# Rorisis/Co-Occ

Hardware: AMD Instinct MI355X
Metric: samples/sec (6-cam frame + sweep -> occ+render), 200x200x16 grid (higher is better)
Workload: dtype f32 (split-f16 products, fp32 accumulate)

## Files before the change

co_occ_amd/csrc/gemm_h2.hip:

```cpp
#include <stdlib.h>
#include <string.h>
#include <type_traits>

#include "conv_k.h"

#include "h2_rows.h"

typedef float f32x16 __attribute__((ext_vector_type(16)));
typedef _Float16 f16x8 __attribute__((ext_vector_type(8)));

__device__ __forceinline__ void glds16_(const void* g, void* l) {
  __builtin_amdgcn_global_load_lds((const __attribute__((address_space(1))) void*)g, (__attribute__((address_space(3))) void*)l,
                                   16, 0, 0);
}

__device__ __forceinline__ void h2_epilogue_vec(const ConvK& p, size_t orow, int n, f32x4 v) {
  if (p.res_mode == 3) v = v + *(const f32x4*)(p.res + orow * p.res_stride + n);
  if (p.scale) v = v * *(const f32x4*)(p.scale + n);
  if (p.bias) v = v + *(const f32x4*)(p.bias + n);
  if (p.res_mode == 1) v = v + *(const f32x4*)(p.res + orow * p.res_stride + n);
  if (p.relu && (p.relu == 1 || n < p.relu)) { v[0] = fmaxf(v[0], 0.f); v[1] = fmaxf(v[1], 0.f); v[2] = fmaxf(v[2], 0.f); v[3] = fmaxf(v[3], 0.f); }
  if (p.res_mode == 2) v = v * *(const f32x4*)(p.res + orow * p.res_stride + n);
  if (p.out_h2) { store_h2(p.out, orow, p.out_stride, n, v); h2_guard(p.h2_flag, v); }
  else *(f32x4*)(p.out + orow * p.out_stride + n) = v;
// ... 492 lines not shown
    p2(STC{}, I1{});
    H2_FENCE();
  };
  if (nsteps > 0) {
    issueA(0);
    loadB(I0{});
  }
  __syncthreads();
  if (nsteps > 0) {
    load_frag(I0{}, I0{}, I0{});
    if (TERMS == 1) load_frag(I1{}, I0{}, I1{});
  }
  for (int st = 0; st < nsteps; st += 2) {
    step(I0{}, st + 1 < nsteps);
    if (st + 1 < nsteps) step(I1{}, st + 2 < nsteps);
  }

  const int nb = n0 + wave * 32 + 4 * h;
  const float alpha = p.alpha_dev ? p.alpha * *p.alpha_dev : p.alpha, lo = TERMS == 3 ? alpha * (1.f / H2_LO_SCALE) : 0.f;
  if (p.splitk > 1) {
#pragma unroll
    for (int i = 0; i < TM; ++i) {
      const int m = m0 + i * 32 + li;
      if (m >= p.M) continue;
      float* o = p.ws + ((size_t)blockIdx.y * p.M + m) * p.Npad + nb;
#pragma unroll
      for (int j = 0; j < 4; ++j) {
        f32x4 v;
#pragma unroll
        for (int e = 0; e < 4; ++e) v[e] = (TERMS == 3 ? hh[i][4 * j + e] * alpha + xx[i][4 * j + e] * lo : hh[i][4 * j + e] * alpha);
        if (p.tile_sem) st_agent(o + 8 * j, v);
        else *(f32x4*)(o + 8 * j) = v;
      }
    }
    if (p.tile_sem && h2_splitk_arrive(p, mtile * p.ntiles + nt)) h2_splitk_reduce<TM>(p, m0, nb, li);
  } else {
    const bool vec = (p.Cout & 3) == 0 && (p.out_stride & 3) == 0 && (!p.res || (p.res_stride & 3) == 0);
#pragma unroll
    for (int i = 0; i < TM; ++i) {
      const int m = m0 + i * 32 + li;
      if (m >= p.M) continue;
      const size_t orow = p.out_rows ? (size_t)p.out_rows[m] : (size_t)m;
#pragma unroll
      for (int j = 0; j < 4; ++j) {
        const int n = nb + 8 * j;
        if (n >= p.Cout) continue;
        f32x4 v;
#pragma unroll
        for (int e = 0; e < 4; ++e) v[e] = (TERMS == 3 ? hh[i][4 * j + e] * alpha + xx[i][4 * j + e] * lo : hh[i][4 * j + e] * alpha);
        if (vec) {
          h2_epilogue_vec(p, orow, n, v);
        } else {
#pragma unroll
          for (int e = 0; e < 4; ++e)
            if (n + e < p.Cout) p.out[orow * p.out_stride + n + e] = epilogue(p, v[e], n + e, orow);
        }
      }
    }
  }
}

template <int NCW>
__global__ __launch_bounds__(256, NCW == 4 ? 3 : 2) void k_gemm_h2n(ConvK p) {
  constexpr int BM = NCW == 4 ? 64 : 256, TM = NCW == 2 ? 4 : 2, NJ = BM / 32;
  constexpr unsigned STAGE = BM * 128;
  __shared__ __attribute__((aligned(16))) char As[2 * BM * 128];

  const int mtiles = (p.M + BM - 1) / BM;
  const int mtile = blockIdx.x;
  if (mtile >= mtiles) return;
  const int m0 = mtile * BM;
  if (p.M_dev) {
    p.M = min(p.M, *p.M_dev);
    if (m0 >= p.M) return;
  }
  const int tid = threadIdx.x;
  const int wave = __builtin_amdgcn_readfirstlane(tid >> 6), lane = tid & 63;
  const int li = lane & 31, h = lane >> 5;
  const int srow = lane >> 3, slot = lane & 7;
  const int colblk = NCW == 4 ? wave : (NCW == 2 ? (wave & 1) : 0);
  const int rowbase = NCW == 4 ? 0 : (NCW == 2 ? (wave >> 1) * 128 : wave * 64);
  const int taps = p.taps;
  const long long rowbytes = (long long)p.in_stride * 4;
  const char* inb = (const char*)p.in;
  const char* zrow = (const char*)p.zrow;
  const unsigned aq = (unsigned)((slot ^ ((4 * (wave & 1) + (srow >> 1)) & 7)) * 16);
  int rix[NJ];
#pragma unroll
  for (int j = 0; j < NJ; ++j) {
    const int m = m0 + (j * 4 + wave) * 8 + srow;
    rix[j] = m < p.M ? m : -1;
  }
  const int nsteps = p.total_iters;
  int ckc = 0, ct = 0;
  const long long wstep = (long long)(p.Npad >> 5) * 4096;
  const char* wcur = (const char*)p.w + (long long)colblk * 4096 + lane * 16;
  const int gstride = p.gstride;
  int tnext[NJ];
  auto tload = [&]() {
#pragma unroll
    for (int j = 0; j < NJ; ++j) tnext[j] = rix[j] >= 0 ? p.gather[(size_t)ct * gstride + rix[j]] : -1;
  };
  if (nsteps > 0) tload();
  auto issueA = [&](int buf) {
    const long long coff = (long long)ckc * 128 + aq;
#pragma unroll
    for (int j = 0; j < NJ; ++j) {
      const char* src = tnext[j] >= 0 ? inb + ((long long)tnext[j] * rowbytes + coff) : zrow;
      glds16_(src, &As[buf * STAGE + (j * 4 + wave) * 8 * 128]);
    }
    if (++ct == taps) { ct = 0; ++ckc; }
    tload();
  };
  f16x8 breg[2][2][2];
  auto loadB = [&](auto bufc) {
    constexpr int B_ = decltype(bufc)::value;
#pragma unroll
    for (int s = 0; s < 2; ++s)
#pragma unroll
      for (int pl = 0; pl < 2; ++pl) breg[B_][s][pl] = *(const f16x8*)(wcur + (s * 2 + pl) * 1024);
    wcur += wstep;
  };
  unsigned fragoff[4];
#pragma unroll
  for (int q = 0; q < 4; ++q) {
    const int sl = (q & 1) * 4 + 2 * (q >> 1) + h;
    fragoff[q] = (rowbase + li) * 128 + ((sl ^ ((li >> 1) & 7)) << 4);
  }
  f16x8 fr[2][TM];
  auto load_frag = [&](auto bufc, auto stagec, auto qc) {
    constexpr int BUF = decltype(bufc)::value, ST = decltype(stagec)::value, Q = decltype(qc)::value;
#pragma unroll
    for (int i = 0; i < TM; ++i) fr[BUF][i] = *(const f16x8*)&As[fragoff[Q] + (ST * STAGE + i * 4096)];
  };
  auto load_plane = [&](auto planec, auto stagec, auto sc) {
    constexpr int PL = decltype(planec)::value, S_ = decltype(sc)::value;
    load_frag(planec, stagec, std::integral_constant<int, 2 * S_ + PL>{});
  };
  f32x16 hh[TM], xx[TM];
#pragma unroll
  for (int i = 0; i < TM; ++i)
#pragma unroll
    for (int r = 0; r < 16; ++r) { hh[i][r] = 0.f; xx[i][r] = 0.f; }
  auto p01 = [&](auto setc, auto sc) {
    constexpr int B_ = decltype(setc)::value, S_ = decltype(sc)::value;
#pragma unroll
    for (int i = 0; i < TM; ++i) hh[i] = __builtin_amdgcn_mfma_f32_32x32x16_f16(breg[B_][S_][0], fr[0][i], hh[i], 0, 0, 0);
#pragma unroll
    for (int i = 0; i < TM; ++i) xx[i] = __builtin_amdgcn_mfma_f32_32x32x16_f16(breg[B_][S_][1], fr[0][i], xx[i], 0, 0, 0);
  };
  auto p2 = [&](auto setc, auto sc) {
    constexpr int B_ = decltype(setc)::value, S_ = decltype(sc)::value;
#pragma unroll
    for (int i = 0; i < TM; ++i) xx[i] = __builtin_amdgcn_mfma_f32_32x32x16_f16(breg[B_][S_][0], fr[1][i], xx[i], 0, 0, 0);
  };
  using I0 = std::integral_constant<int, 0>; using I1 = std::integral_constant<int, 1>;
  auto step = [&](auto stc, bool more) {
    constexpr int ST = decltype(stc)::value;
    using STC = std::integral_constant<int, ST>; using SNC = std::integral_constant<int, ST ^ 1>;
    if (more) { issueA(ST ^ 1); loadB(SNC{}); }
    load_plane(I1{}, STC{}, I0{});
    p01(STC{}, I0{});
    H2_FENCE();
    load_plane(I0{}, STC{}, I1{});
    p2(STC{}, I0{});
    H2_FENCE();
    load_plane(I1{}, STC{}, I1{});
    p01(STC{}, I1{});
    H2_FENCE();
    __syncthreads();
    if (more) load_plane(I0{}, SNC{}, I0{});
    p2(STC{}, I1{});
    H2_FENCE();
  };
  if (nsteps > 0) {
    issueA(0);
    loadB(I0{});
  }
  __syncthreads();
  if (nsteps > 0) load_frag(I0{}, I0{}, I0{});
  for (int st = 0; st < nsteps; st += 2) {
    step(I0{}, st + 1 < nsteps);
    if (st + 1 < nsteps) step(I1{}, st + 2 < nsteps);
  }

  const int nb = colblk * 32 + 4 * h;
  const float alpha = p.alpha_dev ? p.alpha * *p.alpha_dev : p.alpha, lo = alpha * (1.f / H2_LO_SCALE);
  const bool vec = (p.Cout & 3) == 0 && (p.out_stride & 3) == 0 && (!p.res || (p.res_stride & 3) == 0);
#pragma unroll
  for (int i = 0; i < TM; ++i) {
    const int m = m0 + rowbase + i * 32 + li;
    if (m >= p.M) continue;
    const size_t orow = p.out_rows ? (size_t)p.out_rows[m] : (size_t)m;
#pragma unroll
    for (int j = 0; j < 4; ++j) {
      const int n = nb + 8 * j;
      if (n >= p.Cout) continue;
      f32x4 v;
#pragma unroll
      for (int e = 0; e < 4; ++e) v[e] = hh[i][4 * j + e] * alpha + xx[i][4 * j + e] * lo;
      if (vec) {
        h2_epilogue_vec(p, orow, n, v);
      } else {
#pragma unroll
        for (int e = 0; e < 4; ++e)
          if (n + e < p.Cout) p.out[orow * p.out_stride + n + e] = epilogue(p, v[e], n + e, orow);
      }
    }
  }
}

template <int NCH>
__global__ __launch_bounds__(256, 2) void k_gemm_h2p(ConvK p) {
  constexpr int BM = 128, TM = 4;
  constexpr unsigned STAGE = BM * 128;
  __shared__ __attribute__((aligned(16))) char As[NCH * BM * 128];
  const int id = blockIdx.x;
  int mtile, nt, slot_ = id >> 3;
  if (p.mtiles_per_xcd > 0) {
    const int xcd = id & 7;
    const int mt_local = slot_ / p.ntiles;
    nt = slot_ - mt_local * p.ntiles;
    mtile = xcd * p.mtiles_per_xcd + mt_local;
    if (mt_local >= p.mtiles_per_xcd || mtile >= p.mtiles) return;
  } else {
    mtile = id / p.ntiles;
    nt = id - mtile * p.ntiles;
  }
  const int m0 = mtile * BM, n0 = nt * 128;
  const int tid = threadIdx.x;
  const int wave = __builtin_amdgcn_readfirstlane(tid >> 6), lane = tid & 63;
  const int li = lane & 31, h = lane >> 5;
  const int srow = lane >> 3, slot = lane & 7;
  const long long rowbytes = (long long)p.in_stride * 4;
  const char* inb = (const char*)p.in;
  const char* zrow = (const char*)p.zrow;
  const unsigned aq = (unsigned)((slot ^ ((4 * (wave & 1) + (srow >> 1)) & 7)) * 16);
#pragma unroll
  for (int c = 0; c < NCH; ++c)
#pragma unroll
    for (int j = 0; j < 4; ++j) {
      const int m = m0 + (j * 4 + wave) * 8 + srow;
      const char* src = m < p.M ? inb + ((long long)m * rowbytes + c * 128 + aq) : zrow;
      glds16_(src, &As[c * STAGE + (j * 4 + wave) * 8 * 128]);
    }
  f16x8 breg[NCH][2][2];
  const long long wstep = (long long)(p.Npad >> 5) * 4096;
  const char* wcur = (const char*)p.w + (long long)((n0 >> 5) + wave) * 4096 + lane * 16;
#pragma unroll
  for (int c = 0; c < NCH; ++c)
#pragma unroll
    for (int s2 = 0; s2 < 2; ++s2)
#pragma unroll
      for (int pl = 0; pl < 2; ++pl) breg[c][s2][pl] = *(const f16x8*)(wcur + c * wstep + (s2 * 2 + pl) * 1024);
  unsigned fragoff[4];
#pragma unroll
  for (int q = 0; q < 4; ++q) {
    const int sl = (q & 1) * 4 + 2 * (q >> 1) + h;
    fragoff[q] = li * 128 + ((sl ^ ((li >> 1) & 7)) << 4);
  }
  f32x16 hh[TM], xx[TM];
#pragma unroll
  for (int i = 0; i < TM; ++i)
#pragma unroll
    for (int r = 0; r < 16; ++r) { hh[i][r] = 0.f; xx[i][r] = 0.f; }
  __syncthreads();
#pragma unroll
  for (int c = 0; c < NCH; ++c) {
#pragma unroll
    for (int s2 = 0; s2 < 2; ++s2) {
      f16x8 fhi[TM], flo[TM];
#pragma unroll
      for (int i = 0; i < TM; ++i) {
        fhi[i] = *(const f16x8*)&As[fragoff[2 * s2 + 0] + (c * STAGE + i * 4096)];
        flo[i] = *(const f16x8*)&As[fragoff[2 * s2 + 1] + (c * STAGE + i * 4096)];
      }
#pragma unroll
      for (int i = 0; i < TM; ++i) hh[i] = __builtin_amdgcn_mfma_f32_32x32x16_f16(breg[c][s2][0], fhi[i], hh[i], 0, 0, 0);
#pragma unroll
      for (int i = 0; i < TM; ++i) xx[i] = __builtin_amdgcn_mfma_f32_32x32x16_f16(breg[c][s2][1], fhi[i], xx[i], 0, 0, 0);
#pragma unroll
      for (int i = 0; i < TM; ++i) xx[i] = __builtin_amdgcn_mfma_f32_32x32x16_f16(breg[c][s2][0], flo[i], xx[i], 0, 0, 0);
      H2_FENCE();
    }
  }
  const int nb = n0 + wave * 32 + 4 * h;
  const float alpha = p.alpha_dev ? p.alpha * *p.alpha_dev : p.alpha, lo = alpha * (1.f / H2_LO_SCALE);
#pragma unroll
  for (int i = 0; i < TM; ++i) {
    const int m = m0 + i * 32 + li;
    if (m >= p.M) continue;
#pragma unroll
    for (int j = 0; j < 4; ++j) {
      const int n = nb + 8 * j;
      if (n >= p.Cout) continue;
      f32x4 v;
#pragma unroll
      for (int e = 0; e < 4; ++e) v[e] = hh[i][4 * j + e] * alpha + xx[i][4 * j + e] * lo;
      h2_epilogue_vec(p, (size_t)m, n, v);
    }
  }
}

static int* g_h2_flag = nullptr;
int coocc_h2_flag_ptr(int** out) {
  if (!g_h2_flag) {
    void* p = nullptr;
    COOCC_HIP(hipHostMalloc(&p, 64, hipHostMallocMapped | hipHostMallocCoherent));
    memset(p, 0, 64);
    g_h2_flag = (int*)p;
  }
  *out = g_h2_flag;
  return COOCC_OK;
}
extern "C" int coocc_h2_overflow(int reset) {
  if (!g_h2_flag) return 0;
  const int v = *(volatile int*)g_h2_flag != 0;
  if (reset) *(volatile int*)g_h2_flag = 0;
  return v;
}
extern "C" int coocc_device_fault(int reset) {
  if (!g_h2_flag) return 0;
  const int v = ((volatile int*)g_h2_flag)[1];
  if (reset) ((volatile int*)g_h2_flag)[1] = 0;
  return v;
}

int coocc_launch_h2(ConvK& k, const coocc_conv_desc* d, hipStream_t s) {
  const bool one = d->mfma_dtype == 4;
  const int kc = one ? 64 : 32;
  COOCC_CHECK_ARG(d->Cin % kc == 0 && d->in_stride % kc == 0, "conv_fwd: H2 operands need Cin and in_stride % 32 == 0 (f16 operands: % 64)");
  COOCC_CHECK_ARG(!one || (d->wgroup_rows == 0 && !d->out_h2), "conv_fwd: the one-term f16 path has no weight groups / H2 output");
  COOCC_CHECK_ARG(d->wgroup_rows == 0 || d->wgroup_rows % 128 == 0, "conv_fwd: wgroup_rows must be a multiple of 128");
  const bool table = d->gather != nullptr;
  const bool zshare = !table && !d->out_rows && !d->M_dev && k.stride == 1 && k.Xo == k.Xi && k.Yo == k.Yi && k.Zo == k.Zi && k.kz >= 1 && k.kz <= 3 &&
                      (k.taps > 1 || d->wgroup_rows > 0);
  COOCC_CHECK_ARG(zshare || d->wgroup_rows == 0, "conv_fwd: weight groups need the stride-1 same geometry");
  k.kchunks = d->Cin / kc;
  k.total_iters = k.taps * k.kchunks;
  k.wgroup_floats = (size_t)k.taps * k.kchunks * k.Npad * 32;
  k.out16 = d->out16;
  k.out16_stride = d->out16_stride;
  COOCC_CHECK_ARG(!d->out16 || (d->Cout % 4 == 0 && d->out16_stride % 4 == 0 && !d->out_rows && ((uintptr_t)d->out16 & 7) == 0),
                  "conv_fwd: out16 needs Cout % 4 == 0, out16_stride % 4 == 0, no row scatter");
  k.alpha = d->alpha != 0.f ? d->alpha : 1.f;
  k.alpha_dev = d->alpha_dev;
  k.M_dev = d->M_dev;
  k.out_h2 = d->out_h2;
  COOCC_CHECK_ARG(!d->out_h2 || (d->Cout % 4 == 0 && d->out_stride % 32 == 0 && !d->out_rows),
                  "conv_fwd: out_h2 needs Cout % 4 == 0, out_stride % 32 == 0, no row scatter");
  k.out_h2t = d->out_h2_twin;
  COOCC_CHECK_ARG(!d->out_h2_twin || (!one && d->Cout % 32 == 0 && !d->out_rows && ((uintptr_t)d->out_h2_twin & 15) == 0 && (d->out_stride & 3) == 0 &&
                                      (!d->res || (d->res_stride & 3) == 0)),
                  "conv_fwd: out_h2_twin needs mfma_dtype 3, Cout % 32 == 0, 16-byte aligned rows, no row scatter");
  k.tile_sem = d->tile_sem;
  int rc = coocc_zero_row(&k.zrow);
  if (rc != COOCC_OK) return rc;
  rc = coocc_h2_flag_ptr(&k.h2_flag);
  if (rc != COOCC_OK) return rc;
  k.ntiles = (k.Cout + 127) / 128;
  k.mtiles = (k.M + 127) / 128;
  k.mtiles_per_xcd = k.mtiles >= 64 ? (k.mtiles + 7) / 8 : 0;
  const int gsz = zshare ? k.kz : 1;
  int splitk = d->splitk;
  const long long blocks = (long long)k.mtiles * k.ntiles;
  const int ngroups = k.total_iters / gsz;
  if (splitk <= 0) {
    splitk = 1;
    const bool vec4 = (d->Cout & 3) == 0 && (d->out_stride & 3) == 0 && (!d->res || (d->res_stride & 3) == 0) && (((uintptr_t)d->out) & 15) == 0;
    const bool second_pass_ok = vec4 || (!d->out_h2 && !d->out16 && !d->out_h2_twin);
    static const int target = getenv("COOCC_SPLITK_TARGET") ? atoi(getenv("COOCC_SPLITK_TARGET")) : 512;
    if (blocks < target / 2 && ngroups >= 8 && d->ws && !d->M_dev && (d->tile_sem ? true : (!d->out_rows && second_pass_ok))) {
      splitk = (int)(target / blocks);
      if (splitk > ngroups / 4) splitk = ngroups / 4;
      if (splitk > 64) splitk = 64;
      while (splitk > 1 && (long long)splitk * d->M * k.Npad > d->ws_floats) --splitk;
      if (splitk < 1) splitk = 1;
    }
  }
  int gps = (ngroups + splitk - 1) / splitk;
  k.iters_per_split = gps * gsz;
  k.splitk = (k.total_iters + k.iters_per_split - 1) / k.iters_per_split;
  COOCC_CHECK_ARG(k.splitk == 1 || (d->ws && !d->M_dev && (long long)k.splitk * d->M * k.Npad <= d->ws_floats),
                  "conv_fwd: split-K workspace too small (or split-K with a device row count)");
  COOCC_CHECK_ARG(k.splitk == 1 || d->tile_sem || (!d->out_h2 && !d->out16 && !d->out_h2_twin) ||
                      ((d->Cout & 3) == 0 && (d->out_stride & 3) == 0 && (!d->res || (d->res_stride & 3) == 0) && (((uintptr_t)d->out) & 15) == 0),
                  "conv_fwd: split-K with an H2 / f16 output needs 16-byte aligned rows (Cout, strides % 4 == 0)");
  COOCC_CHECK_ARG(k.splitk == 1 || !d->tile_sem || (long long)k.mtiles * k.ntiles <= d->tile_sem_ints,
                  "conv_fwd: tile_sem holds fewer counters than the launch has output tiles");
  dim3 grid(k.mtiles_per_xcd ? 8 * k.mtiles_per_xcd * k.ntiles : k.mtiles * k.ntiles, k.splitk);
  static const bool pointwise_on = !(getenv("COOCC_H2_POINTWISE") && atoi(getenv("COOCC_H2_POINTWISE")) == 0);
  if (pointwise_on && !zshare && !table && !one && k.taps == 1 && k.stride == 1 && k.px == 0 && k.py == 0 && k.pz == 0 && k.Xo == k.Xi &&
      k.Yo == k.Yi && k.Zo == k.Zi && k.kchunks <= 4 && k.splitk == 1 && !d->M_dev && !d->out_rows && blocks >= 256 &&
      (d->Cout & 3) == 0 && (d->out_stride & 3) == 0 && (!d->res || (d->res_stride & 3) == 0)) {
    switch (k.kchunks) {
      case 1: hipLaunchKernelGGL(k_gemm_h2p<1>, grid, dim3(256), 0, s, k); break;
      case 2: hipLaunchKernelGGL(k_gemm_h2p<2>, grid, dim3(256), 0, s, k); break;
      case 3: hipLaunchKernelGGL(k_gemm_h2p<3>, grid, dim3(256), 0, s, k); break;
      default: hipLaunchKernelGGL(k_gemm_h2p<4>, grid, dim3(256), 0, s, k); break;
    }
    COOCC_LAUNCH_CHECK("k_gemm_h2p");
    return COOCC_OK;
  }
  if (!zshare) {
    if (one) {
      if (table) hipLaunchKernelGGL((k_gemm_h2w<true, 1>), grid, dim3(256), 0, s, k);
      else hipLaunchKernelGGL((k_gemm_h2w<false, 1>), grid, dim3(256), 0, s, k);
    } else {
      const char* narrow_env = getenv("COOCC_H2_NARROW");
      const bool narrow_on = !(narrow_env && atoi(narrow_env) == 0);
      if (narrow_on && table && k.Cout <= 64 && k.ntiles == 1 && k.splitk == 1 && !d->tile_sem && (long long)k.mtiles >= 512) {
        const dim3 gridn((unsigned)((k.M + 255) / 256), 1);
        if (k.Cout <= 32) hipLaunchKernelGGL(k_gemm_h2n<1>, gridn, dim3(256), 0, s, k);
        else hipLaunchKernelGGL(k_gemm_h2n<2>, gridn, dim3(256), 0, s, k);
        COOCC_LAUNCH_CHECK("k_gemm_h2n");
        return COOCC_OK;
      }
      if (narrow_on && table && k.Cout > 96 && k.ntiles == 1 && k.splitk == 1 && !d->tile_sem && (long long)k.mtiles >= 128 && (long long)k.mtiles < 1024) {
        const dim3 gridn((unsigned)((k.M + 63) / 64), 1);
        hipLaunchKernelGGL(k_gemm_h2n<4>, gridn, dim3(256), 0, s, k);
        COOCC_LAUNCH_CHECK("k_gemm_h2n<4>");
        return COOCC_OK;
      }
      if (table) hipLaunchKernelGGL(k_gemm_h2w<true>, grid, dim3(256), 0, s, k);
      else hipLaunchKernelGGL(k_gemm_h2w<false>, grid, dim3(256), 0, s, k);
    }
    COOCC_LAUNCH_CHECK("k_gemm_h2w");
    return COOCC_OK;
  }
  COOCC_CHECK_ARG((long long)d->M < (1ll << 30) && (136ull + 2ull * ((unsigned long long)k.Yi + 2) * k.Zi) * d->in_stride * 4ull < 0xFFFFFF00ull,
                  "conv_fwd: the split-f16 kernel addresses a tile's window with 32-bit byte offsets");
  const bool xy = !(k.kx == 1 && k.ky == 1 && k.px == 0 && k.py == 0);
  if (one) {
    if (k.kz == 3) { if (xy) hipLaunchKernelGGL((k_gemm_h2z<3, true, 0, 1>), grid, dim3(256), 0, s, k); else hipLaunchKernelGGL((k_gemm_h2z<3, false, 0, 1>), grid, dim3(256), 0, s, k); }
    else if (k.kz == 2) { if (xy) hipLaunchKernelGGL((k_gemm_h2z<2, true, 0, 1>), grid, dim3(256), 0, s, k); else hipLaunchKernelGGL((k_gemm_h2z<2, false, 0, 1>), grid, dim3(256), 0, s, k); }
    else { if (xy) hipLaunchKernelGGL((k_gemm_h2z<1, true, 0, 1>), grid, dim3(256), 0, s, k); else hipLaunchKernelGGL((k_gemm_h2z<1, false, 0, 1>), grid, dim3(256), 0, s, k); }
    COOCC_LAUNCH_CHECK("k_gemm_h2z<f16>");
    return COOCC_OK;
  }
  static const int abl = getenv("COOCC_H2_ABLATE") ? atoi(getenv("COOCC_H2_ABLATE")) : 0;
  if (abl && !xy && k.kz == 3) {
    switch (abl) {
      case 1: hipLaunchKernelGGL((k_gemm_h2z<3, false, 1>), grid, dim3(256), 0, s, k); break;
      case 2: hipLaunchKernelGGL((k_gemm_h2z<3, false, 2>), grid, dim3(256), 0, s, k); break;
      case 4: hipLaunchKernelGGL((k_gemm_h2z<3, false, 4>), grid, dim3(256), 0, s, k); break;
      case 8: hipLaunchKernelGGL((k_gemm_h2z<3, false, 8>), grid, dim3(256), 0, s, k); break;
      case 7: hipLaunchKernelGGL((k_gemm_h2z<3, false, 7>), grid, dim3(256), 0, s, k); break;
      case 16: hipLaunchKernelGGL((k_gemm_h2z<3, false, 16>), grid, dim3(256), 0, s, k); break;
      case 24: hipLaunchKernelGGL((k_gemm_h2z<3, false, 24>), grid, dim3(256), 0, s, k); break;
      default: hipLaunchKernelGGL((k_gemm_h2z<3, false, 15>), grid, dim3(256), 0, s, k); break;
    }
    COOCC_LAUNCH_CHECK("k_gemm_h2z<ablation>");
    return COOCC_OK;
  }
  if (!xy) {
    if (k.kz == 3) hipLaunchKernelGGL((k_gemm_h2z<3, false>), grid, dim3(256), 0, s, k);
    else if (k.kz == 2) hipLaunchKernelGGL((k_gemm_h2z<2, false>), grid, dim3(256), 0, s, k);
    else hipLaunchKernelGGL((k_gemm_h2z<1, false>), grid, dim3(256), 0, s, k);
  } else {
    if (k.kz == 3) hipLaunchKernelGGL((k_gemm_h2z<3, true>), grid, dim3(256), 0, s, k);
    else if (k.kz == 2) hipLaunchKernelGGL((k_gemm_h2z<2, true>), grid, dim3(256), 0, s, k);
    else hipLaunchKernelGGL((k_gemm_h2z<1, true>), grid, dim3(256), 0, s, k);
  }
  COOCC_LAUNCH_CHECK("k_gemm_h2z");
  return COOCC_OK;
}

__global__ __launch_bounds__(256) void k_rows_to_h2(const float* __restrict__ in, int in_stride, long long rows, int C, float scale,
                                                     char* __restrict__ out, const int32_t* __restrict__ row_ids,
                                                     const int32_t* __restrict__ n_dev, int* __restrict__ flag,
                                                     const float* __restrict__ scale_dev) {
  if (n_dev) rows = min(rows, (long long)*n_dev);
  if (scale_dev) scale *= *scale_dev;
  const int c8 = C >> 3;
  const long long i = (long long)blockIdx.x * blockDim.x + threadIdx.x;
  if (i >= rows * c8) return;
  const long long r = i / c8;
  const int c = (int)(i - r * c8) * 8;
  const long long sr = row_ids ? (long long)row_ids[r] : r;
  const f32x4 a = *(const f32x4*)(in + sr * in_stride + c), b = *(const f32x4*)(in + sr * in_stride + c + 4);
  f16x8 hi, lo;
#pragma unroll
  for (int e = 0; e < 4; ++e) {
    _Float16 u, v;
    split_h2(a[e] * scale, u, v); hi[e] = u; lo[e] = v;
    split_h2(b[e] * scale, u, v); hi[4 + e] = u; lo[4 + e] = v;
  }
  char* o = out + r * (long long)C * 4 + (c >> 5) * 128 + (c & 31) * 2;
  *(f16x8*)o = hi;
  *(f16x8*)(o + 64) = lo;
  h2_guard(flag, a * scale);
  h2_guard(flag, b * scale);
}

extern "C" int coocc_rows_to_h2_ex(const float* in, int in_stride, int64_t rows, int C, float scale, const float* scale_dev,
                                   void* out_h2, void* stream) {
  COOCC_CHECK_ARG(in && out_h2 && rows >= 0 && C > 0 && C % 32 == 0 && in_stride % 4 == 0 && in_stride >= C, "rows_to_h2: bad args");
  COOCC_CHECK_ARG(((uintptr_t)in & 15) == 0 && ((uintptr_t)out_h2 & 15) == 0, "rows_to_h2: pointers must be 16-byte aligned");
  if (rows == 0) return COOCC_OK;
  int* flag = nullptr;
  if (coocc_h2_flag_ptr(&flag) != COOCC_OK) return COOCC_EHIP;
  hipLaunchKernelGGL(k_rows_to_h2, dim3(cdiv(rows * (C / 8), 256)), dim3(256), 0, as_stream(stream), in, in_stride, (long long)rows, C,
                     scale, (char*)out_h2, (const int32_t*)nullptr, (const int32_t*)nullptr, flag, scale_dev);
  COOCC_LAUNCH_CHECK("k_rows_to_h2");
  return COOCC_OK;
}

extern "C" int coocc_rows_to_h2(const float* in, int in_stride, int64_t rows, int C, float scale, void* out_h2, void* stream) {
  return coocc_rows_to_h2_ex(in, in_stride, rows, C, scale, nullptr, out_h2, stream);
}

extern "C" int coocc_rows_to_h2_gather(const float* in, int in_stride, const int32_t* row_ids, int64_t n_cap, const int32_t* n_dev,
                                       int C, float scale, void* out_h2, void* stream) {
  COOCC_CHECK_ARG(in && out_h2 && row_ids && n_cap >= 0 && C > 0 && C % 32 == 0 && in_stride % 4 == 0, "rows_to_h2_gather: bad args");
  COOCC_CHECK_ARG(((uintptr_t)in & 15) == 0 && ((uintptr_t)out_h2 & 15) == 0, "rows_to_h2_gather: pointers must be 16-byte aligned");
  if (n_cap == 0) return COOCC_OK;
  int* flag = nullptr;
  if (coocc_h2_flag_ptr(&flag) != COOCC_OK) return COOCC_EHIP;
  hipLaunchKernelGGL(k_rows_to_h2, dim3(cdiv(n_cap * (C / 8), 256)), dim3(256), 0, as_stream(stream), in, in_stride, (long long)n_cap, C,
                     scale, (char*)out_h2, row_ids, n_dev, flag, (const float*)nullptr);
  COOCC_LAUNCH_CHECK("k_rows_to_h2");
  return COOCC_OK;
}

__global__ __launch_bounds__(256) void k_rows_to_f16(const float* __restrict__ in, int in_stride, long long rows, int C, _Float16* __restrict__ out) {
  const int c8 = C >> 3;
  const long long i = (long long)blockIdx.x * blockDim.x + threadIdx.x;
  if (i >= rows * c8) return;
  const long long r = i / c8;
  const int c = (int)(i - r * c8) * 8;
  const f32x4 a = *(const f32x4*)(in + r * in_stride + c), b = *(const f32x4*)(in + r * in_stride + c + 4);
  f16x8 o;
#pragma unroll
  for (int e = 0; e < 4; ++e) { o[e] = (_Float16)a[e]; o[4 + e] = (_Float16)b[e]; }
  *(f16x8*)(out + r * C + c) = o;
}

extern "C" int coocc_rows_to_f16(const float* in, int in_stride, int64_t rows, int C, void* out_f16, void* stream) {
  COOCC_CHECK_ARG(in && out_f16 && rows >= 0 && C > 0 && C % 8 == 0 && in_stride % 4 == 0 && in_stride >= C, "rows_to_f16: bad args");
  COOCC_CHECK_ARG(((uintptr_t)in & 15) == 0 && ((uintptr_t)out_f16 & 15) == 0, "rows_to_f16: pointers must be 16-byte aligned");
  if (rows == 0) return COOCC_OK;
  hipLaunchKernelGGL(k_rows_to_f16, dim3(cdiv(rows * (C / 8), 256)), dim3(256), 0, as_stream(stream), in, in_stride, (long long)rows, C,
                     (_Float16*)out_f16);
  COOCC_LAUNCH_CHECK("k_rows_to_f16");
  return COOCC_OK;
}
```

Measured before the change: 266.4.

## Add persistent streaming pointwise H2 GEMM kernel with double-buffered LDS row spans

Adds a persistent pointwise 1x1 GEMM kernel sized to the CU count. Each block owns a contiguous span of rows and streams them through double-buffered LDS via global_load_lds, while the weights, scale and bias stay in registers for the whole span. The launcher now uses this kernel by default when there are more tiles than resident slots, and it also covers Cout widths that are not a multiple of four. The aim is to cut per-tile launch and weight-reload overhead and to overlap loads with MFMA work, at the cost of a fixed-size grid and more register pressure.

```diff
diff --git a/co_occ_amd/csrc/gemm_h2.hip b/co_occ_amd/csrc/gemm_h2.hip
--- a/co_occ_amd/csrc/gemm_h2.hip
+++ b/co_occ_amd/csrc/gemm_h2.hip
@@ -818,6 +818,151 @@
   }
 }
 
+__device__ __forceinline__ void h2_epilogue_vec_sb(const ConvK& p, size_t orow, int n, f32x4 v, f32x4 sc, f32x4 bi) {
+  if (p.res_mode == 3) v = v + *(const f32x4*)(p.res + orow * p.res_stride + n);
+  if (p.scale) v = v * sc;
+  if (p.bias) v = v + bi;
+  if (p.res_mode == 1) v = v + *(const f32x4*)(p.res + orow * p.res_stride + n);
+  if (p.relu && (p.relu == 1 || n < p.relu)) { v[0] = fmaxf(v[0], 0.f); v[1] = fmaxf(v[1], 0.f); v[2] = fmaxf(v[2], 0.f); v[3] = fmaxf(v[3], 0.f); }
+  if (p.res_mode == 2) v = v * *(const f32x4*)(p.res + orow * p.res_stride + n);
+  if (p.out_h2) { store_h2(p.out, orow, p.out_stride, n, v); h2_guard(p.h2_flag, v); }
+  else *(f32x4*)(p.out + orow * p.out_stride + n) = v;
+  if (p.out16) { store_f16(p.out16, orow, p.out16_stride, n, v); h2_guard(p.h2_flag, v); }
+  if (p.out_h2t) { store_h2(p.out_h2t, orow, p.Cout, n, v); h2_guard(p.h2_flag, v); }
+}
+template <int N>
+__device__ __forceinline__ void wait_vmcnt_() { asm volatile("s_waitcnt vmcnt(%0)" ::"n"(N) : "memory"); }
+#define H2_PIN(x) asm volatile("" : "+v"(x))
+
+template <int NCH, int TM, bool VEC>
+__global__ __launch_bounds__(256, TM == 2 ? 2 : 1) void k_gemm_h2ps(ConvK p, int nspans) {
+  constexpr unsigned STAGE = TM * 32 * 128, BUF = NCH * STAGE;
+  __shared__ __attribute__((aligned(16))) char As[2 * BUF];
+  const int id = blockIdx.x;
+  const int slot_ = id >> 3;
+  const int sq = slot_ / p.ntiles, nt = slot_ - sq * p.ntiles;
+  const int span = sq * 8 + (id & 7);
+  const int nblk = (p.M + 31) >> 5;
+  const int per = nblk / nspans, rem = nblk - per * nspans;
+  const int b0 = span * per + (span < rem ? span : rem), b1 = b0 + per + (span < rem ? 1 : 0);
+  if (b0 >= b1) return;
+  const int r0 = b0 * 32, r1 = b1 * 32 < p.M ? b1 * 32 : p.M;
+  const int nsub = (b1 - b0 + TM - 1) / TM;
+  const int n0 = nt * 128;
+  const int tid = threadIdx.x;
+  const int wave = __builtin_amdgcn_readfirstlane(tid >> 6), lane = tid & 63;
+  const int li = lane & 31, h = lane >> 5;
+  const int srow = lane >> 3, slot = lane & 7;
+  const long long rowbytes = (long long)p.in_stride * 4;
+  const char* inb = (const char*)p.in;
+  const char* zrow = (const char*)p.zrow;
+  const unsigned aq = (unsigned)((slot ^ ((4 * (wave & 1) + (srow >> 1)) & 7)) * 16);
+  auto request = [&](int t, unsigned buf) {
+    const int mb = r0 + t * (TM * 32);
+#pragma unroll
+    for (int c = 0; c < NCH; ++c)
+#pragma unroll
+      for (int j = 0; j < TM; ++j) {
+        const int m = mb + (j * 4 + wave) * 8 + srow;
+        const char* src = m < r1 ? inb + ((long long)m * rowbytes + c * 128 + aq) : zrow;
+        glds16_(src, &As[buf + c * STAGE + (j * 4 + wave) * 8 * 128]);
+      }
+  };
+  request(0, 0);
+  f16x8 breg[NCH][2][2];
+  const long long wstep = (long long)(p.Npad >> 5) * 4096;
+  const char* wcur = (const char*)p.w + (long long)((n0 >> 5) + wave) * 4096 + lane * 16;
+#pragma unroll
+  for (int c = 0; c < NCH; ++c)
+#pragma unroll
+    for (int s2 = 0; s2 < 2; ++s2)
+#pragma unroll
+      for (int pl = 0; pl < 2; ++pl) breg[c][s2][pl] = *(const f16x8*)(wcur + c * wstep + (s2 * 2 + pl) * 1024);
+  const int nb = n0 + wave * 32 + 4 * h;
+  f32x4 sc[4], bi[4];
+#pragma unroll
+  for (int j = 0; j < 4; ++j) {
+    const bool in = VEC && nb + 8 * j < p.Cout;
+    sc[j] = p.scale && in ? *(const f32x4*)(p.scale + nb + 8 * j) : f32x4{0.f, 0.f, 0.f, 0.f};
+    bi[j] = p.bias && in ? *(const f32x4*)(p.bias + nb + 8 * j) : f32x4{0.f, 0.f, 0.f, 0.f};
+  }
+  float alpha = p.alpha_dev ? p.alpha * *p.alpha_dev : p.alpha;
+  unsigned fragoff[4];
+#pragma unroll
+  for (int q = 0; q < 4; ++q) {
+    const int sl = (q & 1) * 4 + 2 * (q >> 1) + h;
+    fragoff[q] = li * 128 + ((sl ^ ((li >> 1) & 7)) << 4);
+  }
+#pragma unroll
+  for (int c = 0; c < NCH; ++c)
+#pragma unroll
+    for (int s2 = 0; s2 < 2; ++s2) { H2_PIN(breg[c][s2][0]); H2_PIN(breg[c][s2][1]); }
+#pragma unroll
+  for (int j = 0; j < 4; ++j) { H2_PIN(sc[j]); H2_PIN(bi[j]); }
+  H2_PIN(alpha);
+  const float lo = alpha * (1.f / H2_LO_SCALE);
+  const bool cols_full = n0 + wave * 32 + 32 <= p.Cout;
+  wait_vmcnt_<0>();
+  __builtin_amdgcn_s_barrier();
+#pragma unroll 1
+  for (int t = 0; t < nsub; ++t) {
+    const unsigned cur = (t & 1) ? BUF : 0u;
+    const bool more = t + 1 < nsub;
+    if (more) request(t + 1, cur ^ BUF);
+    f32x16 hh[TM], xx[TM];
+#pragma unroll
+    for (int i = 0; i < TM; ++i)
+#pragma unroll
+      for (int r = 0; r < 16; ++r) { hh[i][r] = 0.f; xx[i][r] = 0.f; }
+#pragma unroll
+    for (int c = 0; c < NCH; ++c) {
+#pragma unroll
+      for (int s2 = 0; s2 < 2; ++s2) {
+        f16x8 fhi[TM], flo[TM];
+#pragma unroll
+        for (int i = 0; i < TM; ++i) {
+          fhi[i] = *(const f16x8*)&As[cur + fragoff[2 * s2 + 0] + (c * STAGE + i * 4096)];
+          flo[i] = *(const f16x8*)&As[cur + fragoff[2 * s2 + 1] + (c * STAGE + i * 4096)];
+        }
+#pragma unroll
+        for (int i = 0; i < TM; ++i) hh[i] = __builtin_amdgcn_mfma_f32_32x32x16_f16(breg[c][s2][0], fhi[i], hh[i], 0, 0, 0);
+#pragma unroll
+        for (int i = 0; i < TM; ++i) xx[i] = __builtin_amdgcn_mfma_f32_32x32x16_f16(breg[c][s2][1], fhi[i], xx[i], 0, 0, 0);
+#pragma unroll
+        for (int i = 0; i < TM; ++i) xx[i] = __builtin_amdgcn_mfma_f32_32x32x16_f16(breg[c][s2][0], flo[i], xx[i], 0, 0, 0);
+        H2_FENCE();
+      }
+    }
+    const int mb = r0 + t * (TM * 32);
+#pragma unroll
+    for (int i = 0; i < TM; ++i) {
+      const int m = mb + i * 32 + li;
+      if (m >= r1) continue;
+#pragma unroll
+      for (int j = 0; j < 4; ++j) {
+        const int n = nb + 8 * j;
+        if (n >= p.Cout) continue;
+        f32x4 v;
+#pragma unroll
+        for (int e = 0; e < 4; ++e) v[e] = hh[i][4 * j + e] * alpha + xx[i][4 * j + e] * lo;
+        if constexpr (VEC) {
+          h2_epilogue_vec_sb(p, (size_t)m, n, v, sc[j], bi[j]);
+        } else {
+#pragma unroll
+          for (int e = 0; e < 4; ++e)
+            if (n + e < p.Cout) p.out[(size_t)m * p.out_stride + n + e] = epilogue(p, v[e], n + e, (size_t)m);
+        }
+      }
+    }
+    if (more) {
+      if (cols_full && mb + TM * 32 <= r1) {
+        if (p.out_h2t) wait_vmcnt_<12 * TM>(); else wait_vmcnt_<4 * TM>();
+      } else wait_vmcnt_<0>();
+      __builtin_amdgcn_s_barrier();
+    }
+  }
+}
+
 static int* g_h2_flag = nullptr;
 int coocc_h2_flag_ptr(int** out) {
   if (!g_h2_flag) {
@@ -840,6 +985,15 @@
   const int v = ((volatile int*)g_h2_flag)[1];
   if (reset) ((volatile int*)g_h2_flag)[1] = 0;
   return v;
+}
+
+static int h2ps_cus() {
+  static const int cus = [] {
+    int dev = 0, n = 0;
+    if (hipGetDevice(&dev) != hipSuccess || hipDeviceGetAttribute(&n, hipDeviceAttributeMultiprocessorCount, dev) != hipSuccess || n <= 0) n = 256;
+    return n;
+  }();
+  return cus;
 }
 
 int coocc_launch_h2(ConvK& k, const coocc_conv_desc* d, hipStream_t s) {
@@ -905,18 +1059,42 @@
   COOCC_CHECK_ARG(k.splitk == 1 || !d->tile_sem || (long long)k.mtiles * k.ntiles <= d->tile_sem_ints,
                   "conv_fwd: tile_sem holds fewer counters than the launch has output tiles");
   dim3 grid(k.mtiles_per_xcd ? 8 * k.mtiles_per_xcd * k.ntiles : k.mtiles * k.ntiles, k.splitk);
-  static const bool pointwise_on = !(getenv("COOCC_H2_POINTWISE") && atoi(getenv("COOCC_H2_POINTWISE")) == 0);
-  if (pointwise_on && !zshare && !table && !one && k.taps == 1 && k.stride == 1 && k.px == 0 && k.py == 0 && k.pz == 0 && k.Xo == k.Xi &&
-      k.Yo == k.Yi && k.Zo == k.Zi && k.kchunks <= 4 && k.splitk == 1 && !d->M_dev && !d->out_rows && blocks >= 256 &&
-      (d->Cout & 3) == 0 && (d->out_stride & 3) == 0 && (!d->res || (d->res_stride & 3) == 0)) {
-    switch (k.kchunks) {
-      case 1: hipLaunchKernelGGL(k_gemm_h2p<1>, grid, dim3(256), 0, s, k); break;
-      case 2: hipLaunchKernelGGL(k_gemm_h2p<2>, grid, dim3(256), 0, s, k); break;
-      case 3: hipLaunchKernelGGL(k_gemm_h2p<3>, grid, dim3(256), 0, s, k); break;
-      default: hipLaunchKernelGGL(k_gemm_h2p<4>, grid, dim3(256), 0, s, k); break;
-    }
-    COOCC_LAUNCH_CHECK("k_gemm_h2p");
-    return COOCC_OK;
+  const char* pw_env = getenv("COOCC_H2_POINTWISE");
+  const int pw = pw_env ? atoi(pw_env) : 2;
+  if (pw != 0 && !zshare && !table && !one && k.taps == 1 && k.stride == 1 && k.px == 0 && k.py == 0 && k.pz == 0 && k.Xo == k.Xi &&
+      k.Yo == k.Yi && k.Zo == k.Zi && k.kchunks <= 4 && k.splitk == 1 && !d->M_dev && !d->out_rows && (blocks >= 256 || pw >= 3)) {
+    const bool vec4 = (d->Cout & 3) == 0 && (d->out_stride & 3) == 0 && (!d->res || (d->res_stride & 3) == 0);
+    static const int tm = getenv("COOCC_H2_STREAM_ROWS") && atoi(getenv("COOCC_H2_STREAM_ROWS")) == 128 ? 4 : 2;
+    const int slots = h2ps_cus() * (tm == 2 ? 2 : 1);
+    if (pw == 3 || (pw == 2 && blocks > slots)) {
+      int nspans = (slots / k.ntiles) & ~7;
+      if (nspans < 8) nspans = 8;
+      const dim3 grids((unsigned)(nspans * k.ntiles));
+#define H2PS_LAUNCH(NCH)                                                                                       \
+  if (tm == 2 && vec4) hipLaunchKernelGGL((k_gemm_h2ps<NCH, 2, true>), grids, dim3(256), 0, s, k, nspans);       \
+  else if (tm == 2) hipLaunchKernelGGL((k_gemm_h2ps<NCH, 2, false>), grids, dim3(256), 0, s, k, nspans);         \
+  else if (vec4) hipLaunchKernelGGL((k_gemm_h2ps<NCH, 4, true>), grids, dim3(256), 0, s, k, nspans);             \
+  else hipLaunchKernelGGL((k_gemm_h2ps<NCH, 4, false>), grids, dim3(256), 0, s, k, nspans)
+      switch (k.kchunks) {
+        case 1: H2PS_LAUNCH(1); break;
+        case 2: H2PS_LAUNCH(2); break;
+        case 3: H2PS_LAUNCH(3); break;
+        default: H2PS_LAUNCH(4); break;
+      }
+#undef H2PS_LAUNCH
+      COOCC_LAUNCH_CHECK("k_gemm_h2ps");
+      return COOCC_OK;
+    }
+    if (vec4) {
+      switch (k.kchunks) {
+        case 1: hipLaunchKernelGGL(k_gemm_h2p<1>, grid, dim3(256), 0, s, k); break;
+        case 2: hipLaunchKernelGGL(k_gemm_h2p<2>, grid, dim3(256), 0, s, k); break;
+        case 3: hipLaunchKernelGGL(k_gemm_h2p<3>, grid, dim3(256), 0, s, k); break;
+        default: hipLaunchKernelGGL(k_gemm_h2p<4>, grid, dim3(256), 0, s, k); break;
+      }
+      COOCC_LAUNCH_CHECK("k_gemm_h2p");
+      return COOCC_OK;
+    }
   }
   if (!zshare) {
     if (one) {
```

Result: no change. 264.9 (-0.6%).
